# rangasaishreyas/FacePoseGenerator

Hardware: AMD Instinct MI355X
Metric: 512x512 images/sec/node, SD-2.1-base 30-step DDPM CFG=5.0 + LoRA (higher is better)
Workload: dtype f16

## Files before the change

faceposegenerator_amd/csrc/idb_attn.hip:

```cpp
#include "idb_common.h"
#include <stdlib.h>
#include <type_traits>

namespace {

constexpr int KS = 144;
constexpr int VS = 192;
constexpr int KV_TILE = 64;
constexpr int K_BYTES = KV_TILE * KS, V_BYTES = KV_TILE * VS, BUF_BYTES = K_BYTES + V_BYTES;

template <typename T, int NW, int KSPLIT = 1>
__global__ __launch_bounds__(64 * NW) void attn_kernel(const T* __restrict__ q, int q_ld, const T* __restrict__ k,
                                                   const T* __restrict__ v, int kv_ld, T* __restrict__ out, int out_ld,
                                                   int n_q, int n_kv, int n_kv_alloc, float scale_log2e, int causal) {
    using V8 = typename Op<T>::v8;
    using V4 = typename Op<T>::v4;
    constexpr int MERGE_BYTES = KSPLIT == 2 ? 34 * (NW / KSPLIT) * 64 * 4 : 0;
    __shared__ __attribute__((aligned(16))) char smem[2 * BUF_BYTES > MERGE_BYTES ? 2 * BUF_BYTES : MERGE_BYTES];

    const int tid = threadIdx.x, lane = tid & 63, wave = tid >> 6;
    const int r = lane & 31, h = lane >> 5;
    const int head = blockIdx.y, b = blockIdx.z;
    constexpr int NWQ = NW / KSPLIT, NKB = 2 / KSPLIT;
    const int wq = wave % NWQ, kb0 = (wave / NWQ) * NKB;
    const int q0 = blockIdx.x * (32 * NWQ) + wq * 32;

    V8 qf[4];
    {
        const int qr = min(q0 + r, n_q - 1);
        const T* qp = q + ((long long)b * n_q + qr) * q_ld + head * 64 + 8 * h;
#pragma unroll
        for (int s = 0; s < 4; ++s) qf[s] = *(const V8*)(qp + 16 * s);
    }

    const T* kbase = k + (long long)b * n_kv_alloc * kv_ld + head * 64;
    const T* vbase = v + (long long)b * n_kv_alloc * kv_ld + head * 64;
    const int ntiles = (n_kv + KV_TILE - 1) / KV_TILE;

    constexpr int PF = 1;
    constexpr int CH = NW >= 8 ? 1 : 8 / NW, RSTEP = NW >= 8 ? 64 : 8 * NW;
    const bool stager = NW <= 8 || tid < 512;
    const int srow = tid >> 3, schunk = tid & 7;
    V8 kreg[PF][CH], vreg[PF][CH];
    auto gload = [&](auto SET, int t) {
        constexpr int st = decltype(SET)::value;
        if (!stager) return;
#pragma unroll
        for (int i = 0; i < CH; ++i) {
            const int row = min(t * KV_TILE + srow + RSTEP * i, n_kv - 1);
            kreg[st][i] = *(const V8*)(kbase + (long long)row * kv_ld + schunk * 8);
            vreg[st][i] = *(const V8*)(vbase + (long long)row * kv_ld + schunk * 8);
        }
    };
    auto lstore = [&](auto SET, int buf) {
        constexpr int st = decltype(SET)::value;
        if (!stager) return;
        char* kb_ = smem + buf * BUF_BYTES;
        char* vb_ = kb_ + K_BYTES;
#pragma unroll
        for (int i = 0; i < CH; ++i) {
            *(V8*)(kb_ + (srow + RSTEP * i) * KS + schunk * 16) = kreg[st][i];
            *(V8*)(vb_ + (srow + RSTEP * i) * VS + schunk * 16) = vreg[st][i];
        }
    };
    using Set0 = std::integral_constant<int, 0>;
    using Set1 = std::integral_constant<int, PF - 1>;

    f32x16 oacc[2];
#pragma unroll
    for (int d = 0; d < 2; ++d)
#pragma unroll
        for (int i = 0; i < 16; ++i) oacc[d][i] = 0.f;
    float m_run = -INFINITY, l_run = 0.f;

    gload(Set0{}, 0);
    if constexpr (PF == 2) {
        if (ntiles > 1) gload(Set1{}, 1);
    }
    lstore(Set0{}, 0);
    __syncthreads();

    const int tr_row = 4 * h + ((lane & 15) >> 2);
    const int tr_col = 16 * ((lane >> 4) & 1) + 4 * (lane & 3);

    auto tile_body = [&](auto TAIL, auto PAR, int t) {
        const int cur = t & 1;
        using Next = std::integral_constant<int, PF == 2 ? 1 - decltype(PAR)::value : 0>;
        if constexpr (PF == 2) {
            if (t + 2 < ntiles) gload(PAR, t + 2);
        } else {
            if (t + 1 < ntiles) gload(PAR, t + 1);
        }
        const char* kt = smem + cur * BUF_BYTES;
        const char* vt = kt + K_BYTES;

        f32x16 sacc[NKB];
#pragma unroll
        for (int kb = 0; kb < NKB; ++kb) {
            const f32x16 zero = {0.f, 0.f, 0.f, 0.f, 0.f, 0.f, 0.f, 0.f, 0.f, 0.f, 0.f, 0.f, 0.f, 0.f, 0.f, 0.f};
#pragma unroll
            for (int s = 0; s < 4; ++s) {
                const V8 kf = *(const V8*)(kt + ((kb0 + kb) * 32 + r) * KS + (2 * s + h) * 16);
                sacc[kb] = Op<T>::mfma32(kf, qf[s], s == 0 ? zero : sacc[kb]);
            }
        }
        float mx = -INFINITY;
#pragma unroll
        for (int kb = 0; kb < NKB; ++kb)
#pragma unroll
            for (int i = 0; i < 16; ++i) {
                if constexpr (decltype(TAIL)::value) {
                    const int key = t * KV_TILE + (kb0 + kb) * 32 + (i & 3) + 8 * (i >> 2) + 4 * h;
                    if (key >= n_kv || (causal && key > q0 + r)) sacc[kb][i] = -INFINITY;
                }
                mx = fmaxf(mx, sacc[kb][i]);
            }
        mx = fmaxf(mx, __shfl_xor(mx, 32, 64));
        const float m_new = fmaxf(m_run, mx);
        const float alpha = __builtin_amdgcn_exp2f((m_run - m_new) * scale_log2e);
        const bool grew = m_new > m_run;
        m_run = m_new;
        const float mb = m_new * scale_log2e;
        float rs = 0.f;
        V8 pf[NKB][2];
#pragma unroll
        for (int kb = 0; kb < NKB; ++kb)
#pragma unroll
            for (int s2 = 0; s2 < 2; ++s2)
#pragma unroll
                for (int j = 0; j < 8; ++j) {
                    const float pv = __builtin_amdgcn_exp2f(__builtin_fmaf(sacc[kb][8 * s2 + j], scale_log2e, -mb));
                    rs += pv;
                    pf[kb][s2][j] = from_f32<T>(pv);
                }
        l_run = l_run * alpha + rs;
        if (__builtin_amdgcn_ballot_w64(grew) != 0) {
#pragma unroll
            for (int d = 0; d < 2; ++d)
#pragma unroll
                for (int i = 0; i < 16; ++i) oacc[d][i] *= alpha;
        }

#pragma unroll
        for (int kb = 0; kb < NKB; ++kb)
#pragma unroll
            for (int s2 = 0; s2 < 2; ++s2) {
                const int base_row = (kb0 + kb) * 32 + 16 * s2 + tr_row;
#pragma unroll
                for (int d = 0; d < 2; ++d) {
                    const char* va = vt + base_row * VS + (d * 32 + tr_col) * 2;
                    const V4 lo = Op<T>::ds_read_tr(va);
                    const V4 hi = Op<T>::ds_read_tr(va + 8 * VS);
                    V8 vf;
#pragma unroll
                    for (int j = 0; j < 4; ++j) {
                        vf[j] = lo[j];
                        vf[j + 4] = hi[j];
                    }
                    oacc[d] = Op<T>::mfma32(vf, pf[kb][s2], oacc[d]);
                }
            }

        if (t + 1 < ntiles) lstore(Next{}, cur ^ 1);
        __syncthreads();
    };
    auto run = [&](auto TAIL, int t) {
        if constexpr (PF == 2) {
            if (t & 1) tile_body(TAIL, Set1{}, t);
            else tile_body(TAIL, Set0{}, t);
        } else {
            tile_body(TAIL, Set0{}, t);
        }
    };
    const int nfull = causal ? 0 : n_kv / KV_TILE;
    for (int t = 0; t < nfull; ++t) run(std::false_type{}, t);
    for (int t = nfull; t < ntiles; ++t) run(std::true_type{}, t);

    if constexpr (KSPLIT == 2) {
        float* xs = (float*)smem;
        constexpr int LN = NWQ * 64;
        const int slot = wq * 64 + lane;
        if (kb0 != 0) {
            xs[slot] = m_run;
            xs[LN + slot] = l_run;
#pragma unroll
            for (int d = 0; d < 2; ++d)
#pragma unroll
                for (int i = 0; i < 16; ++i) xs[(2 + d * 16 + i) * LN + slot] = oacc[d][i];
        }
        __syncthreads();
        if (kb0 != 0) return;
        const float m_o = xs[slot], l_o = xs[LN + slot];
        const float m_new = fmaxf(m_run, m_o);
        const float a_s = m_run == -INFINITY ? 0.f : __builtin_amdgcn_exp2f((m_run - m_new) * scale_log2e);
        const float a_o = m_o == -INFINITY ? 0.f : __builtin_amdgcn_exp2f((m_o - m_new) * scale_log2e);
        l_run = l_run * a_s + l_o * a_o;
#pragma unroll
        for (int d = 0; d < 2; ++d)
#pragma unroll
            for (int i = 0; i < 16; ++i) oacc[d][i] = oacc[d][i] * a_s + xs[(2 + d * 16 + i) * LN + slot] * a_o;
    }
    const float l_tot = l_run + __shfl_xor(l_run, 32, 64);
    const float inv = 1.0f / l_tot;
    if (q0 + r < n_q) {
        T* op = out + ((long long)b * n_q + q0 + r) * out_ld + head * 64 + 4 * h;
#pragma unroll
        for (int d = 0; d < 2; ++d)
#pragma unroll
            for (int g4 = 0; g4 < 4; ++g4) {
                V4 pk;
#pragma unroll
                for (int e = 0; e < 4; ++e) pk[e] = from_f32<T>(oacc[d][4 * g4 + e] * inv);
                *(V4*)(op + d * 32 + 8 * g4) = pk;
            }
    }
}

}

extern "C" int idb_attention(const void* q, int32_t q_ld, const void* k, const void* v, int32_t kv_ld, void* out,
                             int32_t out_ld, int32_t batch, int32_t heads, int32_t n_q, int32_t n_kv, int32_t n_kv_alloc,
                             float scale, int32_t causal, int32_t dtype, void* stream) {
    IDB_REQUIRE(idb_is_operand_dtype(dtype), "idb_attention: dtype must be bf16/f16");
    IDB_REQUIRE(q && k && v && out, "idb_attention: null pointer");
    IDB_REQUIRE(idb_aligned16(q) && idb_aligned16(k) && idb_aligned16(v) && idb_aligned16(out), "idb_attention: unaligned pointer");
    IDB_REQUIRE(batch > 0 && heads > 0 && n_q > 0 && n_kv > 0 && n_kv_alloc >= n_kv, "idb_attention: bad dims");
    IDB_REQUIRE(q_ld % 8 == 0 && kv_ld % 8 == 0 && out_ld % 4 == 0, "idb_attention: row strides must be multiples of 8 (q,kv) / 4 (out)");
    IDB_REQUIRE(q_ld >= heads * 64 && kv_ld >= heads * 64 && out_ld >= heads * 64, "idb_attention: row stride < heads*64");
    IDB_REQUIRE(batch <= 65535 && heads <= 65535, "idb_attention: grid too large");
    IDB_REQUIRE(!causal || n_q == n_kv, "idb_attention: causal needs n_q == n_kv");
    const float sl2 = scale * 1.44269504088896340736f;
    hipStream_t st = (hipStream_t)stream;
    const long long blocks128 = (long long)((n_q + 127) / 128) * heads * batch;
    const bool small = blocks128 < 128;
    static const int env_ks = [] { const char* e = getenv("IDB_ATTN_KSPLIT"); return e ? atoi(e) : 1; }();
    const bool ksplit = env_ks && !small && !causal && blocks128 < 512 && n_kv >= 512;
    const long long blocks192 = (long long)((n_q + 191) / 192) * heads * batch;
    const bool wide = ksplit && env_ks != 2 && blocks128 > 256 && blocks192 <= 256;
    const dim3 grid(wide ? (n_q + 191) / 192 : (n_q + (small ? 63 : 127)) / (small ? 64 : 128), heads, batch);
#define IDB_ATTN_LAUNCH(T, NW)                                                                                          \
    hipLaunchKernelGGL((attn_kernel<T, NW>), grid, dim3(64 * NW), 0, st, (const T*)q, q_ld, (const T*)k, (const T*)v, kv_ld, \
                       (T*)out, out_ld, n_q, n_kv, n_kv_alloc, sl2, causal)
#define IDB_ATTN_LAUNCH_KS(T)                                                                                           \
    do {                                                                                                                \
        if (wide)                                                                                                       \
            hipLaunchKernelGGL((attn_kernel<T, 12, 2>), grid, dim3(768), 0, st, (const T*)q, q_ld, (const T*)k, (const T*)v, kv_ld, \
                               (T*)out, out_ld, n_q, n_kv, n_kv_alloc, sl2, causal);                                  \
        else                                                                                                            \
            hipLaunchKernelGGL((attn_kernel<T, 8, 2>), grid, dim3(512), 0, st, (const T*)q, q_ld, (const T*)k, (const T*)v, kv_ld,  \
                               (T*)out, out_ld, n_q, n_kv, n_kv_alloc, sl2, causal);                                  \
    } while (0)
    if (dtype == IDB_BF16) {
        if (small) IDB_ATTN_LAUNCH(__bf16, 2);
        else if (ksplit) IDB_ATTN_LAUNCH_KS(__bf16);
        else IDB_ATTN_LAUNCH(__bf16, 4);
    } else {
        if (small) IDB_ATTN_LAUNCH(_Float16, 2);
        else if (ksplit) IDB_ATTN_LAUNCH_KS(_Float16);
        else IDB_ATTN_LAUNCH(_Float16, 4);
    }
#undef IDB_ATTN_LAUNCH
#undef IDB_ATTN_LAUNCH_KS
    IDB_CHECK_LAUNCH("idb_attention");
    return IDB_OK;
}
```

Baseline: 6.753.

## Software-pipeline QK of next tile with softmax/PV and lazy rescaling in k-split attention

Adds a pipelined variant of the k-split flash-attention kernel. It computes QK^T for tile t+1 while softmax and PV run for tile t, staggers the K and V global loads and LDS stores, and only rescales the output accumulator when the running max grows by more than a threshold (FA4-style lazy rescale). It also adds a 96-row, 6-wave launch configuration and generalises the staging-thread count. The aim is to overlap MFMA work with exp/softmax and memory latency, at the cost of more registers (two score buffers) and some added complexity in the numerics.

```diff
diff --git a/faceposegenerator_amd/csrc/idb_attn.hip b/faceposegenerator_amd/csrc/idb_attn.hip
--- a/faceposegenerator_amd/csrc/idb_attn.hip
+++ b/faceposegenerator_amd/csrc/idb_attn.hip
@@ -9,7 +9,9 @@
 constexpr int KV_TILE = 64;
 constexpr int K_BYTES = KV_TILE * KS, V_BYTES = KV_TILE * VS, BUF_BYTES = K_BYTES + V_BYTES;
 
-template <typename T, int NW, int KSPLIT = 1>
+constexpr float RESCALE_LOG2 = 8.f;
+
+template <typename T, int NW, int KSPLIT, bool PIPE>
 __global__ __launch_bounds__(64 * NW) void attn_kernel(const T* __restrict__ q, int q_ld, const T* __restrict__ k,
                                                    const T* __restrict__ v, int kv_ld, T* __restrict__ out, int out_ld,
                                                    int n_q, int n_kv, int n_kv_alloc, float scale_log2e, int causal) {
@@ -37,34 +39,39 @@
     const T* vbase = v + (long long)b * n_kv_alloc * kv_ld + head * 64;
     const int ntiles = (n_kv + KV_TILE - 1) / KV_TILE;
 
-    constexpr int PF = 1;
-    constexpr int CH = NW >= 8 ? 1 : 8 / NW, RSTEP = NW >= 8 ? 64 : 8 * NW;
-    const bool stager = NW <= 8 || tid < 512;
+    constexpr int NS = NW >= 8 ? 8 : NW >= 4 ? 4 : 2;
+    constexpr int CH = 8 / NS, RSTEP = 8 * NS;
+    const bool stager = NW == NS || tid < 64 * NS;
     const int srow = tid >> 3, schunk = tid & 7;
-    V8 kreg[PF][CH], vreg[PF][CH];
-    auto gload = [&](auto SET, int t) {
-        constexpr int st = decltype(SET)::value;
+    V8 kreg[CH], vreg[CH];
+    auto kload = [&](int t) {
         if (!stager) return;
 #pragma unroll
         for (int i = 0; i < CH; ++i) {
             const int row = min(t * KV_TILE + srow + RSTEP * i, n_kv - 1);
-            kreg[st][i] = *(const V8*)(kbase + (long long)row * kv_ld + schunk * 8);
-            vreg[st][i] = *(const V8*)(vbase + (long long)row * kv_ld + schunk * 8);
-        }
-    };
-    auto lstore = [&](auto SET, int buf) {
-        constexpr int st = decltype(SET)::value;
+            kreg[i] = *(const V8*)(kbase + (long long)row * kv_ld + schunk * 8);
+        }
+    };
+    auto vload = [&](int t) {
+        if (!stager) return;
+#pragma unroll
+        for (int i = 0; i < CH; ++i) {
+            const int row = min(t * KV_TILE + srow + RSTEP * i, n_kv - 1);
+            vreg[i] = *(const V8*)(vbase + (long long)row * kv_ld + schunk * 8);
+        }
+    };
+    auto kstore = [&](int buf) {
         if (!stager) return;
         char* kb_ = smem + buf * BUF_BYTES;
-        char* vb_ = kb_ + K_BYTES;
-#pragma unroll
-        for (int i = 0; i < CH; ++i) {
-            *(V8*)(kb_ + (srow + RSTEP * i) * KS + schunk * 16) = kreg[st][i];
-            *(V8*)(vb_ + (srow + RSTEP * i) * VS + schunk * 16) = vreg[st][i];
-        }
-    };
-    using Set0 = std::integral_constant<int, 0>;
-    using Set1 = std::integral_constant<int, PF - 1>;
+#pragma unroll
+        for (int i = 0; i < CH; ++i) *(V8*)(kb_ + (srow + RSTEP * i) * KS + schunk * 16) = kreg[i];
+    };
+    auto vstore = [&](int buf) {
+        if (!stager) return;
+        char* vb_ = smem + buf * BUF_BYTES + K_BYTES;
+#pragma unroll
+        for (int i = 0; i < CH; ++i) *(V8*)(vb_ + (srow + RSTEP * i) * VS + schunk * 16) = vreg[i];
+    };
 
     f32x16 oacc[2];
 #pragma unroll
@@ -72,29 +79,13 @@
 #pragma unroll
         for (int i = 0; i < 16; ++i) oacc[d][i] = 0.f;
     float m_run = -INFINITY, l_run = 0.f;
-
-    gload(Set0{}, 0);
-    if constexpr (PF == 2) {
-        if (ntiles > 1) gload(Set1{}, 1);
-    }
-    lstore(Set0{}, 0);
-    __syncthreads();
+    float alpha_run = 1.f;
 
     const int tr_row = 4 * h + ((lane & 15) >> 2);
     const int tr_col = 16 * ((lane >> 4) & 1) + 4 * (lane & 3);
 
-    auto tile_body = [&](auto TAIL, auto PAR, int t) {
-        const int cur = t & 1;
-        using Next = std::integral_constant<int, PF == 2 ? 1 - decltype(PAR)::value : 0>;
-        if constexpr (PF == 2) {
-            if (t + 2 < ntiles) gload(PAR, t + 2);
-        } else {
-            if (t + 1 < ntiles) gload(PAR, t + 1);
-        }
-        const char* kt = smem + cur * BUF_BYTES;
-        const char* vt = kt + K_BYTES;
-
-        f32x16 sacc[NKB];
+    auto qk = [&](int buf, f32x16 (&sacc)[NKB]) {
+        const char* kt = smem + buf * BUF_BYTES;
 #pragma unroll
         for (int kb = 0; kb < NKB; ++kb) {
             const f32x16 zero = {0.f, 0.f, 0.f, 0.f, 0.f, 0.f, 0.f, 0.f, 0.f, 0.f, 0.f, 0.f, 0.f, 0.f, 0.f, 0.f};
@@ -104,25 +95,72 @@
                 sacc[kb] = Op<T>::mfma32(kf, qf[s], s == 0 ? zero : sacc[kb]);
             }
         }
-        float mx = -INFINITY;
-#pragma unroll
-        for (int kb = 0; kb < NKB; ++kb)
-#pragma unroll
-            for (int i = 0; i < 16; ++i) {
-                if constexpr (decltype(TAIL)::value) {
+    };
+    auto softmax_max = [&](f32x16 (&sacc)[NKB], int t, bool masked) {
+        if (masked) {
+#pragma unroll
+            for (int kb = 0; kb < NKB; ++kb)
+#pragma unroll
+                for (int i = 0; i < 16; ++i) {
                     const int key = t * KV_TILE + (kb0 + kb) * 32 + (i & 3) + 8 * (i >> 2) + 4 * h;
                     if (key >= n_kv || (causal && key > q0 + r)) sacc[kb][i] = -INFINITY;
                 }
-                mx = fmaxf(mx, sacc[kb][i]);
-            }
+        }
+        if constexpr (!PIPE) {
+            float mx = -INFINITY;
+#pragma unroll
+            for (int kb = 0; kb < NKB; ++kb)
+#pragma unroll
+                for (int i = 0; i < 16; ++i) mx = fmaxf(mx, sacc[kb][i]);
+            mx = fmaxf(mx, __shfl_xor(mx, 32, 64));
+            const float m_new = fmaxf(m_run, mx);
+            alpha_run = __builtin_amdgcn_exp2f((m_run - m_new) * scale_log2e);
+            const bool grew = m_new > m_run;
+            m_run = m_new;
+            if (__builtin_amdgcn_ballot_w64(grew) != 0) {
+#pragma unroll
+                for (int d = 0; d < 2; ++d)
+#pragma unroll
+                    for (int i = 0; i < 16; ++i) oacc[d][i] *= alpha_run;
+            }
+            return;
+        }
+        float mx2[2] = {-INFINITY, -INFINITY};
+#pragma unroll
+        for (int kb = 0; kb < NKB; ++kb)
+#pragma unroll
+            for (int i = 0; i < 16; ++i) mx2[(kb * 16 + i) * 2 / (16 * NKB)] = fmaxf(mx2[(kb * 16 + i) * 2 / (16 * NKB)], sacc[kb][i]);
+        float mx = fmaxf(mx2[0], mx2[1]);
         mx = fmaxf(mx, __shfl_xor(mx, 32, 64));
-        const float m_new = fmaxf(m_run, mx);
-        const float alpha = __builtin_amdgcn_exp2f((m_run - m_new) * scale_log2e);
-        const bool grew = m_new > m_run;
-        m_run = m_new;
-        const float mb = m_new * scale_log2e;
-        float rs = 0.f;
-        V8 pf[NKB][2];
+        if (__builtin_amdgcn_ballot_w64((mx - m_run) * scale_log2e > RESCALE_LOG2) != 0) {
+            const float m_new = fmaxf(m_run, mx);
+            const float alpha = m_new == m_run ? 1.f : __builtin_amdgcn_exp2f((m_run - m_new) * scale_log2e);
+            m_run = m_new;
+            l_run *= alpha;
+#pragma unroll
+            for (int d = 0; d < 2; ++d)
+#pragma unroll
+                for (int i = 0; i < 16; ++i) oacc[d][i] *= alpha;
+        }
+    };
+    auto softmax_exp = [&](const f32x16 (&sacc)[NKB], V8 (&pf)[NKB][2]) {
+        const float mb = m_run * scale_log2e;
+        if constexpr (!PIPE) {
+            float rs = 0.f;
+#pragma unroll
+            for (int kb = 0; kb < NKB; ++kb)
+#pragma unroll
+                for (int s2 = 0; s2 < 2; ++s2)
+#pragma unroll
+                    for (int j = 0; j < 8; ++j) {
+                        const float pv = __builtin_amdgcn_exp2f(__builtin_fmaf(sacc[kb][8 * s2 + j], scale_log2e, -mb));
+                        rs += pv;
+                        pf[kb][s2][j] = from_f32<T>(pv);
+                    }
+            l_run = l_run * alpha_run + rs;
+            return;
+        }
+        float rs[4] = {0.f, 0.f, 0.f, 0.f};
 #pragma unroll
         for (int kb = 0; kb < NKB; ++kb)
 #pragma unroll
@@ -130,17 +168,13 @@
 #pragma unroll
                 for (int j = 0; j < 8; ++j) {
                     const float pv = __builtin_amdgcn_exp2f(__builtin_fmaf(sacc[kb][8 * s2 + j], scale_log2e, -mb));
-                    rs += pv;
+                    rs[j & 3] += pv;
                     pf[kb][s2][j] = from_f32<T>(pv);
                 }
-        l_run = l_run * alpha + rs;
-        if (__builtin_amdgcn_ballot_w64(grew) != 0) {
-#pragma unroll
-            for (int d = 0; d < 2; ++d)
-#pragma unroll
-                for (int i = 0; i < 16; ++i) oacc[d][i] *= alpha;
-        }
-
+        l_run += (rs[0] + rs[1]) + (rs[2] + rs[3]);
+    };
+    auto pv = [&](int buf, const V8 (&pf)[NKB][2]) {
+        const char* vt = smem + buf * BUF_BYTES + K_BYTES;
 #pragma unroll
         for (int kb = 0; kb < NKB; ++kb)
 #pragma unroll
@@ -160,21 +194,65 @@
                     oacc[d] = Op<T>::mfma32(vf, pf[kb][s2], oacc[d]);
                 }
             }
-
-        if (t + 1 < ntiles) lstore(Next{}, cur ^ 1);
+    };
+
+    const int nfull = causal ? 0 : n_kv / KV_TILE;
+    if constexpr (PIPE) {
+        kload(0);
+        vload(0);
+        kstore(0);
+        vstore(0);
+        kload(1);
+        kstore(1);
         __syncthreads();
-    };
-    auto run = [&](auto TAIL, int t) {
-        if constexpr (PF == 2) {
-            if (t & 1) tile_body(TAIL, Set1{}, t);
-            else tile_body(TAIL, Set0{}, t);
-        } else {
-            tile_body(TAIL, Set0{}, t);
-        }
-    };
-    const int nfull = causal ? 0 : n_kv / KV_TILE;
-    for (int t = 0; t < nfull; ++t) run(std::false_type{}, t);
-    for (int t = nfull; t < ntiles; ++t) run(std::true_type{}, t);
+        f32x16 sA[NKB], sB[NKB];
+        qk(0, sA);
+        __syncthreads();
+        auto step = [&](f32x16 (&cur)[NKB], f32x16 (&nxt)[NKB], int t) {
+            softmax_max(cur, t, t >= nfull);
+            kload(t + 2);
+            vload(t + 1);
+            qk((t + 1) & 1, nxt);
+            V8 pf[NKB][2];
+            softmax_exp(cur, pf);
+            pv(t & 1, pf);
+            kstore(t & 1);
+            vstore((t + 1) & 1);
+            __syncthreads();
+        };
+        for (int t = 0;; t += 2) {
+            step(sA, sB, t);
+            if (t + 1 >= ntiles) break;
+            step(sB, sA, t + 1);
+            if (t + 2 >= ntiles) break;
+        }
+    } else {
+        kload(0);
+        vload(0);
+        kstore(0);
+        vstore(0);
+        __syncthreads();
+        auto tile = [&](int t, auto MASKED) {
+            const int cur = t & 1;
+            if (t + 1 < ntiles) {
+                kload(t + 1);
+                vload(t + 1);
+            }
+            f32x16 sacc[NKB];
+            qk(cur, sacc);
+            V8 pf[NKB][2];
+            softmax_max(sacc, t, decltype(MASKED)::value);
+            softmax_exp(sacc, pf);
+            pv(cur, pf);
+            if (t + 1 < ntiles) {
+                kstore(cur ^ 1);
+                vstore(cur ^ 1);
+            }
+            __syncthreads();
+        };
+        for (int t = 0; t < nfull; ++t) tile(t, std::false_type{});
+        for (int t = nfull; t < ntiles; ++t) tile(t, std::true_type{});
+    }
 
     if constexpr (KSPLIT == 2) {
         float* xs = (float*)smem;
@@ -236,31 +314,27 @@
     static const int env_ks = [] { const char* e = getenv("IDB_ATTN_KSPLIT"); return e ? atoi(e) : 1; }();
     const bool ksplit = env_ks && !small && !causal && blocks128 < 512 && n_kv >= 512;
     const long long blocks192 = (long long)((n_q + 191) / 192) * heads * batch;
-    const bool wide = ksplit && env_ks != 2 && blocks128 > 256 && blocks192 <= 256;
-    const dim3 grid(wide ? (n_q + 191) / 192 : (n_q + (small ? 63 : 127)) / (small ? 64 : 128), heads, batch);
-#define IDB_ATTN_LAUNCH(T, NW)                                                                                          \
-    hipLaunchKernelGGL((attn_kernel<T, NW>), grid, dim3(64 * NW), 0, st, (const T*)q, q_ld, (const T*)k, (const T*)v, kv_ld, \
-                       (T*)out, out_ld, n_q, n_kv, n_kv_alloc, sl2, causal)
-#define IDB_ATTN_LAUNCH_KS(T)                                                                                           \
+    const long long blocks96 = (long long)((n_q + 95) / 96) * heads * batch;
+    const int rows = !ksplit ? (small ? 64 : 128)
+                     : blocks128 > 256 && blocks192 <= 256 ? 192
+                     : blocks128 <= 256 && blocks96 <= 256 && blocks96 > blocks128 ? 96 : 128;
+    const dim3 grid((n_q + rows - 1) / rows, heads, batch);
+#define IDB_ATTN_LAUNCH(T, NW, KSPLIT)                                                                                  \
+    hipLaunchKernelGGL((attn_kernel<T, NW, KSPLIT, KSPLIT == 2>), grid, dim3(64 * NW), 0, st, (const T*)q, q_ld, (const T*)k,  \
+                       (const T*)v, kv_ld, (T*)out, out_ld, n_q, n_kv, n_kv_alloc, sl2, causal)
+#define IDB_ATTN_DISPATCH(T)                                                                                            \
     do {                                                                                                                \
-        if (wide)                                                                                                       \
-            hipLaunchKernelGGL((attn_kernel<T, 12, 2>), grid, dim3(768), 0, st, (const T*)q, q_ld, (const T*)k, (const T*)v, kv_ld, \
-                               (T*)out, out_ld, n_q, n_kv, n_kv_alloc, sl2, causal);                                  \
-        else                                                                                                            \
-            hipLaunchKernelGGL((attn_kernel<T, 8, 2>), grid, dim3(512), 0, st, (const T*)q, q_ld, (const T*)k, (const T*)v, kv_ld,  \
-                               (T*)out, out_ld, n_q, n_kv, n_kv_alloc, sl2, causal);                                  \
+        if (!ksplit) {                                                                                                  \
+            if (small) IDB_ATTN_LAUNCH(T, 2, 1);                                                                        \
+            else IDB_ATTN_LAUNCH(T, 4, 1);                                                                              \
+        } else if (rows == 192) IDB_ATTN_LAUNCH(T, 12, 2);                                                              \
+        else if (rows == 96) IDB_ATTN_LAUNCH(T, 6, 2);                                                                  \
+        else IDB_ATTN_LAUNCH(T, 8, 2);                                                                                  \
     } while (0)
-    if (dtype == IDB_BF16) {
-        if (small) IDB_ATTN_LAUNCH(__bf16, 2);
-        else if (ksplit) IDB_ATTN_LAUNCH_KS(__bf16);
-        else IDB_ATTN_LAUNCH(__bf16, 4);
-    } else {
-        if (small) IDB_ATTN_LAUNCH(_Float16, 2);
-        else if (ksplit) IDB_ATTN_LAUNCH_KS(_Float16);
-        else IDB_ATTN_LAUNCH(_Float16, 4);
-    }
+    if (dtype == IDB_BF16) IDB_ATTN_DISPATCH(__bf16);
+    else IDB_ATTN_DISPATCH(_Float16);
 #undef IDB_ATTN_LAUNCH
-#undef IDB_ATTN_LAUNCH_KS
+#undef IDB_ATTN_DISPATCH
     IDB_CHECK_LAUNCH("idb_attention");
     return IDB_OK;
 }
```

Measured after the change: 6.810, median of 6. No clear change (+0.8%).
